# tensorflow/recommenders

Hardware: AMD Instinct MI355X
Metric: queries/sec brute-force top-100 (higher is better)
Workload: dtype f32; 1 GPU; BruteForce top-100, 1M-item x dim-64 corpus, batch 8192 (BASELINE.json configs[1]); corpus_rows_total=1000000, corpus_rows_per_gpu=1000000, dim=64, batch=8192, k=100, parallelism=single GPU

## Files before the change

recommenders_amd/csrc/topk_scan16.hip:

```cpp
#include <stdlib.h>

#include <string.h>

#include "common.h"

#ifndef TFRS_SCAN16_ABLATE
#define TFRS_SCAN16_ABLATE 0
#endif
#if TFRS_SCAN16_ABLATE
#ifndef TFRS_ALLOW_ABLATION
#error "TFRS_SCAN16_ABLATE != 0 is a measurement build with wrong results: add -DTFRS_ALLOW_ABLATION to confirm"
#endif
extern "C" int tfrs_ablation_build_scan16(void) { return TFRS_SCAN16_ABLATE; }
#endif
#ifndef TFRS_SCAN16_PEEL
#define TFRS_SCAN16_PEEL 2
#endif

#ifndef TFRS_SCAN16_CLOCKS
#define TFRS_SCAN16_CLOCKS 0
#endif

namespace tfrs {

typedef float f32x16 __attribute__((ext_vector_type(16)));
typedef float f32x4 __attribute__((ext_vector_type(4)));
typedef _Float16 f16x8 __attribute__((ext_vector_type(8)));
typedef _Float16 f16x2 __attribute__((ext_vector_type(2)));
typedef uint32_t u32x4 __attribute__((ext_vector_type(4)));

constexpr int kWaves16 = 8;
constexpr int kThreads16 = kWaves16 * 64;
constexpr int kQG = 2;
static_assert(kWaves16 * kQG * 32 == kScan16QueriesPerWg, "queries per workgroup");

enum Scan16Mode { kModeFilter = 0, kModeMaterialize = 1, kModeBinMax = 2 };

template <int DP>
struct Scan16Geom {
  static constexpr int kSteps = DP / 16;
  static constexpr int kRowB = DP * 2 + 16;
  static constexpr int kStageB = kTileN * kRowB;
  static constexpr int kChunks = kStageB / 16;
  static constexpr int kLoads = (kChunks + kThreads16 - 1) / kThreads16;
  static constexpr int kMetaOff = 2 * kStageB;
  static constexpr int kLdsBytes = 2 * kStageB + 32;
};


template <bool NT = false>
__device__ __forceinline__ void glds_copy16(const char *gsrc_lane, const char *lds_wave_base) {
  const uint32_t m0v = (uint32_t)(uintptr_t)(
      __attribute__((address_space(3))) const char *)lds_wave_base;
  uint32_t m0_saved;
  if constexpr (NT) {
    asm volatile("s_mov_b32 %0, m0\n\ts_mov_b32 m0, %2\n\ts_nop 0\n\t"
                 "global_load_lds_dwordx4 %1, off nt\n\ts_mov_b32 m0, %0"
                 : "=&s"(m0_saved)
                 : "v"(gsrc_lane), "s"(m0v)
                 : "memory");
  } else {
    asm volatile("s_mov_b32 %0, m0\n\ts_mov_b32 m0, %2\n\ts_nop 0\n\t"
                 "global_load_lds_dwordx4 %1, off\n\ts_mov_b32 m0, %0"
                 : "=&s"(m0_saved)
                 : "v"(gsrc_lane), "s"(m0v)
                 : "memory");
  }
}
__device__ __forceinline__ void wait_dma() {
  __builtin_amdgcn_s_waitcnt(0 | (7 << 4) | (15 << 8) | (0 << 14));
}

template <int CHUNKS, int LOADS, bool NT = false>
__device__ __forceinline__ void stage16_glds(const char *gsrc, char *lds_dst, const StageMeta *meta,
                                             char *lds_meta, int tid, int wave) {
#pragma unroll
  for (int i = 0; i < LOADS; ++i) {
    const int ch0 = i * kThreads16 + wave * 64;
    if (ch0 < CHUNKS)
      glds_copy16<NT>(gsrc + (size_t)(i * kThreads16 + tid) * 16, lds_dst + ch0 * 16);
  }
  if (tid == 0) glds_copy16(reinterpret_cast<const char *>(meta), lds_meta);
}

__device__ __forceinline__ f16x8 as_f16x8(u32x4 v) {
  union {
    u32x4 u;
    f16x8 b;
  } x;
  x.u = v;
  return x.b;
}
__device__ __forceinline__ uint32_t cvt_f16x2(float lo, float hi) {
  union {
    f16x2 h;
    uint32_t u;
  } v;
  v.h[0] = (_Float16)lo;
  v.h[1] = (_Float16)hi;
  return v.u;
}
__device__ __forceinline__ float mx3(float a, float b, float c) {
  return __builtin_fmaxf(__builtin_fmaxf(a, b), c);
}
__device__ __forceinline__ float max16(const f32x16 &c) {
  const float a = mx3(c[0], c[1], c[2]), b = mx3(c[3], c[4], c[5]), d = mx3(c[6], c[7], c[8]),
              e = mx3(c[9], c[10], c[11]), f = mx3(c[12], c[13], c[14]);
  return __builtin_fmaxf(mx3(a, b, d), mx3(e, f, c[15]));
}

__device__ __forceinline__ float max8(const f32x4 &c0, const f32x4 &c1) {
  return mx3(mx3(c0[0], c0[1], c0[2]), mx3(c0[3], c1[0], c1[1]), __builtin_fmaxf(c1[2], c1[3]));
}

template <int DP, int MF>
struct Scan16Mfma {
  static_assert(MF == 32 || (MF == 16 && DP >= 32), "the 16x16x32 shape needs 32 features per instruction");
  static constexpr int kQH = 32 / MF;
  static constexpr int kQW = MF;
  static constexpr int kKPer = 512 / MF;
  static constexpr int kKSteps = DP / kKPer;
  static constexpr int kFrags = DP / 16;
  static constexpr int kChain = kQH * kQH * kKSteps;
  static constexpr int kValuPerMfma = (MF == 16 && DP >= 64) ? 2 : 3;
  static constexpr int a_off(int sub, int m, int row_b) {
    return MF == 32 ? sub * 32 * row_b + m * 32
                    : (sub * 32 + 16 * (m / kKSteps)) * row_b + (m % kKSteps) * 64;
  }
};

template <int DP, int MODE, bool NT = false, int MF = 32>
__global__ void __launch_bounds__(kThreads16, DP <= 64 ? 4 : 2) scan16_kernel(const Scan16Args a) {
  using G = Scan16Geom<DP>;
  using M = Scan16Mfma<DP, MF>;
  static_assert(MF == 32 || MODE != kModeFilter, "the first-generation FILTER exists in the 32x32 shape only");
  constexpr int kNS = kQG * M::kQH;
  extern __shared__ __attribute__((aligned(16))) char smem[];

  const int tid = threadIdx.x;
  const int lane = tid & 63;
  const int wave = __builtin_amdgcn_readfirstlane(tid >> 6);
  if (MODE == kModeFilter && a.zero_word && blockIdx.x == 0 && tid == 0) *a.zero_word = 0u;
  if (MODE == kModeFilter && a.zero_aux && blockIdx.x == 0 && tid < 4) a.zero_aux[tid] = 0u;
  const int j = lane & (MF - 1);
  const int h = lane / MF;

  const int nwg = gridDim.x;
  const int bid = blockIdx.x;
  const int q8 = nwg >> 3, r8 = nwg & 7;
  const int xcd = bid & 7, pos = bid >> 3;
  const int logical = (xcd < r8 ? xcd * (q8 + 1) : r8 * (q8 + 1) + (xcd - r8) * q8) + pos;
  const int split = logical / a.n_qtiles;
  const int qt = logical - split * a.n_qtiles;

  const int i0 = split * a.stages_per_split;
  int i1 = i0 + a.stages_per_split;
  if (i1 > a.n_stages) i1 = a.n_stages;
  if (i0 >= i1) return;
  const int nst = i1 - i0;
  const int64_t stride = a.stage_stride;
  const int64_t first_stage = a.stage0 + (int64_t)i0 * stride;

  f16x8 bq[kNS][M::kKSteps];
  float lower[kNS], qk[kNS], qs[kNS], qinv[kNS];
  bool qvalid[kNS];
  int64_t qrow[kNS];
  uint2 *wp[kNS];
  uint32_t mycnt[kNS];
  const bool vec_ok = (a.d == DP) && ((reinterpret_cast<uintptr_t>(a.q) & 15) == 0);
  float4 qlo[kNS][M::kKSteps], qhi[kNS][M::kKSteps];
  int64_t qclampv[kNS];
#pragma unroll
  for (int g = 0; g < kNS; ++g) {
    qrow[g] = (int64_t)qt * kScan16QueriesPerWg + wave * (kQG * 32) + g * M::kQW + j;
    qvalid[g] = qrow[g] < a.nq;
    qclampv[g] = qvalid[g] ? qrow[g] : a.nq - 1;
    qs[g] = a.qscale[qclampv[g]];
  }
  if (vec_ok) {
#pragma unroll
    for (int g = 0; g < kNS; ++g) {
      const float *qp = a.q + qclampv[g] * a.d;
#pragma unroll
      for (int m = 0; m < M::kKSteps; ++m) {
        qlo[g][m] = *reinterpret_cast<const float4 *>(qp + M::kKPer * m + 8 * h);
        qhi[g][m] = *reinterpret_cast<const float4 *>(qp + M::kKPer * m + 8 * h + 4);
      }
    }
  }
#pragma unroll
  for (int g = 0; g < kNS; ++g) {
    const int64_t qclamp = qclampv[g];
    const float *qp = a.q + qclamp * a.d;
    if (!qvalid[g]) qs[g] = 1.0f;
    qinv[g] = 1.0f / qs[g];
#pragma unroll
    for (int m = 0; m < M::kKSteps; ++m) {
      float x[8];
      if (vec_ok) {
        float4 lo = qlo[g][m], hi = qhi[g][m];
        if (!qvalid[g]) lo = hi = make_float4(0.f, 0.f, 0.f, 0.f);
        x[0] = lo.x; x[1] = lo.y; x[2] = lo.z; x[3] = lo.w;
        x[4] = hi.x; x[5] = hi.y; x[6] = hi.z; x[7] = hi.w;
      } else {
#pragma unroll
        for (int i = 0; i < 8; ++i) {
          const int k = M::kKPer * m + 8 * h + i;
          x[i] = (qvalid[g] && k < a.d) ? qp[k] : 0.0f;
        }
      }
      u32x4 w;
#pragma unroll
      for (int i = 0; i < 4; ++i) w[i] = cvt_f16x2(x[2 * i] * qinv[g], x[2 * i + 1] * qinv[g]);
      bq[g][m] = as_f16x8(w);
    }
    lower[g] = __builtin_inff();
    qk[g] = 0.0f;
    if (MODE == kModeFilter) {
      const float lw = a.lower[qclamp], kq = a.qk[qclamp];
      lower[g] = qvalid[g] ? lw : __builtin_inff();
      qk[g] = qvalid[g] ? kq : 0.0f;
    }
    wp[g] = (MODE == kModeFilter)
                ? a.buf + (qrow[g] * (int64_t)a.cap_l) * a.nseg + (2 * split + h)
                : nullptr;
    mycnt[g] = 0;
  }
  const uint32_t row_limit = (uint32_t)a.row_limit;
  const bool wave_active =
      (int64_t)qt * kScan16QueriesPerWg + wave * (kQG * 32) < a.nq;

  static_assert(G::kChunks % 64 == 0, "stage size must be a whole number of wave copies");
  const char *gsrc = a.packed16 + first_stage * (int64_t)G::kStageB;
  const int64_t gstep = stride * (int64_t)G::kStageB;
  const StageMeta *mp = a.meta + first_stage;
  stage16_glds<G::kChunks, G::kLoads, NT>(gsrc, smem, mp, smem + G::kMetaOff, tid, wave);
  wait_dma();
  __syncthreads();

  float binmax[kNS];
#pragma unroll
  for (int g = 0; g < kNS; ++g) binmax[g] = -__builtin_inff();
  for (int st = 0; st < nst; ++st) {
    const char *tile = smem + (st & 1) * G::kStageB;
    const bool more = (st + 1 < nst);
    if (more) {
      stage16_glds<G::kChunks, G::kLoads, NT>(gsrc + (int64_t)(st + 1) * gstep,
                                          smem + ((st + 1) & 1) * G::kStageB,
                                          mp + (int64_t)(st + 1) * stride,
                                          smem + G::kMetaOff + ((st + 1) & 1) * 16, tid, wave);
    }
    const StageMeta sm = *reinterpret_cast<const StageMeta *>(smem + G::kMetaOff + (st & 1) * 16);
    float thr[kNS], unscale[kNS];
#pragma unroll
    for (int g = 0; g < kNS; ++g) {
      thr[g] = (__builtin_fmaf(-qk[g], sm.norm, lower[g]) - kF16Tiny) * qinv[g] * sm.inv_scale;
      unscale[g] = qs[g] * sm.scale;
    }
    if (MODE == kModeBinMax && (st % a.bin_stages) == 0) {
#pragma unroll
      for (int g = 0; g < kNS; ++g) binmax[g] = -__builtin_inff();
    }

    float stagemax[kNS];
#pragma unroll
    for (int g = 0; g < kNS; ++g) stagemax[g] = -__builtin_inff();
    const uint32_t stage_row = (uint32_t)((first_stage + (int64_t)st * stride) * kTileN);
    const char *ap = tile + j * G::kRowB + h * 16;

    if (!wave_active) goto stage_done;
    {
    u32x4 af[2][M::kFrags];
#pragma unroll
    for (int m = 0; m < M::kFrags; ++m) af[0][m] = *reinterpret_cast<const u32x4 *>(ap + M::a_off(0, m, G::kRowB));

    f32x16 acc[kQG];
    f32x4 acc4[kNS][2];
    auto chain = [&](int g, int sub) __attribute__((always_inline)) {
      if constexpr (MF == 16) {
#pragma unroll
        for (int qh = 0; qh < 2; ++qh)
#pragma unroll
          for (int ch = 0; ch < 2; ++ch) acc4[2 * g + qh][ch] = f32x4{0.0f, 0.0f, 0.0f, 0.0f};
#pragma unroll
        for (int m = 0; m < M::kKSteps; ++m)
#pragma unroll
          for (int qh = 0; qh < 2; ++qh)
#pragma unroll
            for (int ch = 0; ch < 2; ++ch)
              acc4[2 * g + qh][ch] = __builtin_amdgcn_mfma_f32_16x16x32_f16(
                  as_f16x8(af[sub & 1][ch * M::kKSteps + m]), bq[2 * g + qh][m], acc4[2 * g + qh][ch], 0, 0, 0);
        return;
      }
#pragma unroll
      for (int r = 0; r < 16; ++r) acc[g][r] = 0.0f;
#pragma unroll
      for (int m = 0; m < G::kSteps; ++m)
        acc[g] = __builtin_amdgcn_mfma_f32_32x32x16_f16(as_f16x8(af[sub & 1][m]), bq[g][m], acc[g], 0, 0, 0);
    };
    auto check = [&](int g, int sub) __attribute__((always_inline)) {
      if constexpr (MF == 16) {
#pragma unroll
        for (int qh = 0; qh < 2; ++qh) {
          const int s = 2 * g + qh;
          if (MODE == kModeMaterialize) {
            if (qvalid[s]) {
              float *drow = a.dense + qrow[s] * a.ld_dense + ((int64_t)(i0 + st) * kTileN + sub * 32 + 4 * h);
#pragma unroll
              for (int ch = 0; ch < 2; ++ch)
                *reinterpret_cast<float4 *>(drow + 16 * ch) =
                    make_float4(acc4[s][ch][0] * unscale[s], acc4[s][ch][1] * unscale[s],
                                acc4[s][ch][2] * unscale[s], acc4[s][ch][3] * unscale[s]);
            }
          } else {
            stagemax[s] = __builtin_fmaxf(stagemax[s], max8(acc4[s][0], acc4[s][1]));
            asm volatile("" : "+v"(stagemax[s]));
          }
        }
        return;
      }
      const f32x16 &c = acc[g];
      if (MODE == kModeMaterialize) {
        if (qvalid[g]) {
          float *drow = a.dense + qrow[g] * a.ld_dense +
                        ((int64_t)(i0 + st) * kTileN + sub * 32 + 4 * h);
#pragma unroll
          for (int g4 = 0; g4 < 4; ++g4)
            *reinterpret_cast<float4 *>(drow + 8 * g4) =
                make_float4(c[4 * g4 + 0] * unscale[g], c[4 * g4 + 1] * unscale[g],
                            c[4 * g4 + 2] * unscale[g], c[4 * g4 + 3] * unscale[g]);
        }
        return;
      }
      const float m0 = max16(c);
      if (MODE == kModeBinMax) {
        stagemax[g] = __builtin_fmaxf(stagemax[g], m0);
        asm volatile("" : "+v"(stagemax[g]));
        return;
      }
      if (__ballot(m0 > thr[g]) != 0ull) {
        const uint32_t rbase = stage_row + sub * 32 + 4u * h;
#pragma unroll
        for (int g4 = 0; g4 < 4; ++g4) {
          const float gm = __builtin_fmaxf(mx3(c[4 * g4], c[4 * g4 + 1], c[4 * g4 + 2]), c[4 * g4 + 3]);
          if (__ballot(gm > thr[g]) == 0ull) continue;
#pragma unroll
          for (int rr = 0; rr < 4; ++rr) {
            const float v = c[4 * g4 + rr];
            const uint32_t row = rbase + rr + 8 * g4;
            if (v > thr[g] && row < row_limit) {
              if (mycnt[g] < a.cap_l) *wp[g] = make_uint2(__float_as_uint(v * unscale[g]), row);
              wp[g] += a.nseg;
              ++mycnt[g];
            }
          }
        }
      }
    };
    auto interleave = [&]() __attribute__((always_inline)) {
#pragma unroll
      for (int i = 0; i < M::kChain; ++i) {
        __builtin_amdgcn_sched_group_barrier(0x008, 1, 0);
        __builtin_amdgcn_sched_group_barrier(0x002, M::kValuPerMfma, 0);
      }
    };

    chain(0, 0);
#pragma unroll
    for (int sub = 0; sub < kTileN / 32; ++sub) {
      if (sub + 1 < kTileN / 32) {
#pragma unroll
        for (int m = 0; m < M::kFrags; ++m)
          af[(sub + 1) & 1][m] =
              *reinterpret_cast<const u32x4 *>(ap + M::a_off(sub + 1, m, G::kRowB));
      }
      __builtin_amdgcn_sched_barrier(0);
      chain(1, sub);
      check(0, sub);
      if (MODE != kModeMaterialize) interleave();
      if (sub + 1 < kTileN / 32) {
        chain(0, sub + 1);
        check(1, sub);
        if (MODE != kModeMaterialize) interleave();
      } else {
        check(1, sub);
      }
    }
    }
  stage_done:
    if (MODE == kModeBinMax && wave_active) {
#pragma unroll
      for (int g = 0; g < kNS; ++g) binmax[g] = __builtin_fmaxf(binmax[g], stagemax[g] * unscale[g]);
      if ((st % a.bin_stages) == a.bin_stages - 1 || st == nst - 1) {
#pragma unroll
        for (int g = 0; g < kNS; ++g) {
          if constexpr (MF == 16) {
            const float v = __builtin_fmaxf(binmax[g], __shfl_xor(binmax[g], 16));
            if (qvalid[g] && (h & 1) == 0)
              a.binmax[qrow[g] * a.ld_binmax + 2 * ((i0 + st) / a.bin_stages) + (h >> 1)] = v;
          } else {
            if (qvalid[g])
              a.binmax[qrow[g] * a.ld_binmax + 2 * ((i0 + st) / a.bin_stages) + h] = binmax[g];
          }
        }
      }
    }
    wait_dma();
    __syncthreads();
  }

  if (MODE == kModeFilter) {
#pragma unroll
    for (int g = 0; g < kNS; ++g)
      if (qvalid[g]) a.cnt[qrow[g] * a.nseg + 2 * split + h] = mycnt[g];
  }
}


template <int DP, int NW, int QG, int SPB = 1, int MF = 32>
struct Scan16FGeom : Scan16Geom<DP> {
  using B = Scan16Geom<DP>;
  static constexpr int kTiles = NW * QG * 32 / kScan16QueriesPerWg;
  static constexpr int kWavesPerTile = NW / kTiles;
  static_assert(kTiles >= 1 && kTiles * kScan16QueriesPerWg == NW * QG * 32, "queries per workgroup");
  static constexpr int kThreads = NW * 64;
  static constexpr int kLoadsF = (B::kChunks + kThreads - 1) / kThreads;
  static constexpr int kQCap = 32;
  static constexpr int kEntB = MF == 16 ? 48 : 80;
  static constexpr int kWaveB = kQCap * kEntB + QG * 64 * 4 + QG * 64 * 16;
  static constexpr int kSlots = 2 * SPB;
  static constexpr int kMetaOffF = kSlots * B::kStageB;
  static constexpr int kQueueOff = (kMetaOffF + kSlots * 16 + 15) / 16 * 16;
  static constexpr int kLdsBytesF = kQueueOff + NW * kWaveB;
  static_assert(kLdsBytesF <= 160 * 1024, "LDS budget");
};

template <int CHUNKS, int LOADS, int THREADS, bool NT = false>
__device__ __forceinline__ void stage16f_glds(const char *gsrc, char *lds_dst, const StageMeta *meta,
                                              char *lds_meta, int tid, int wave) {
#pragma unroll
  for (int i = 0; i < LOADS; ++i) {
    const int ch0 = i * THREADS + wave * 64;
    if (ch0 < CHUNKS)
      glds_copy16<NT>(gsrc + (size_t)(i * THREADS + tid) * 16, lds_dst + ch0 * 16);
  }
  if (tid == 0) glds_copy16(reinterpret_cast<const char *>(meta), lds_meta);
}

__device__ __forceinline__ uint32_t lds_atomic_inc(uint32_t *p) {
  return __hip_atomic_fetch_add(p, 1u, __ATOMIC_RELAXED, __HIP_MEMORY_SCOPE_WAVEFRONT);
}


template <int DP, int NW, int QG, int SPB = 1, bool NT = false, int MF = 32>
__global__ void __launch_bounds__(NW * 64, NW * QG >= 32 ? 1 : (DP <= 64 ? 2 : 1) * NW / 4) scan16f_kernel(const Scan16Args a) {
  using G = Scan16FGeom<DP, NW, QG, SPB, MF>;
  using M = Scan16Mfma<DP, MF>;
  static_assert(MF == 32 || QG == 2, "the 16x16 shape is written for the two-group schedule");
  constexpr int kNS = QG * M::kQH;
  extern __shared__ __attribute__((aligned(16))) char smem[];

  const int tid = threadIdx.x;
  const int lane = tid & 63;
  const int wave = __builtin_amdgcn_readfirstlane(tid >> 6);
  if (a.zero_word && blockIdx.x == 0 && tid == 0) *a.zero_word = 0u;
  if (a.zero_aux && blockIdx.x == 0 && tid < 4) a.zero_aux[tid] = 0u;
  long long clk0 = 0, wall0 = 0;
  if (TFRS_SCAN16_CLOCKS) { clk0 = clock64(); wall0 = wall_clock64(); }
  const int j = lane & (MF - 1);
  const int h = lane / MF;
  const int tj = lane & 31;
  const int th = lane >> 5;

  const int nwg = gridDim.x;
  const int bid = blockIdx.x;
  const int q8 = nwg >> 3, r8 = nwg & 7;
  const int xcd = bid & 7, pos = bid >> 3;
  const int logical = (xcd < r8 ? xcd * (q8 + 1) : r8 * (q8 + 1) + (xcd - r8) * q8) + pos;
  const int n_qgroups = (a.n_qtiles + G::kTiles - 1) / G::kTiles;
  const int split = logical / n_qgroups;
  const int qt = (logical - split * n_qgroups) * G::kTiles + wave / G::kWavesPerTile;
  const int wave_in_tile = wave % G::kWavesPerTile;

  const int i0 = split * a.stages_per_split;
  int i1 = i0 + a.stages_per_split;
  if (i1 > a.n_stages) i1 = a.n_stages;
  if (i0 >= i1) return;
  const int nst = i1 - i0;
  const int64_t first_stage = a.stage0 + (int64_t)i0 * a.stage_stride;

  char *const qbase = smem + G::kQueueOff + wave * G::kWaveB;
  uint32_t *const wcnt = reinterpret_cast<uint32_t *>(qbase + G::kQCap * G::kEntB);
  #pragma unroll
  for (int g = 0; g < QG; ++g) wcnt[g * 64 + lane] = 0u;
  const int64_t q0 = (int64_t)qt * kScan16QueriesPerWg + wave_in_tile * (QG * 32);

  f16x8 bq[kNS][M::kKSteps];
  float4 *const qconst = reinterpret_cast<float4 *>(qbase + G::kQCap * G::kEntB + QG * 64 * 4);
  const bool vec_ok = (a.d == DP) && ((reinterpret_cast<uintptr_t>(a.q) & 15) == 0);
  float4 qlo[kNS][M::kKSteps], qhi[kNS][M::kKSteps];
  float qscv[QG], lowv[QG], qkv[QG];
  float qscb[kNS];
#pragma unroll
  for (int g = 0; g < QG; ++g) {
    const int64_t qrow = q0 + g * 32 + tj;
    const int64_t qclamp = qrow < a.nq ? qrow : a.nq - 1;
    qscv[g] = a.qscale[qclamp];
    lowv[g] = a.lower[qclamp];
    qkv[g] = a.qk[qclamp];
  }
  if constexpr (MF == 16) {
#pragma unroll
    for (int s = 0; s < kNS; ++s) {
      const int64_t qrow = q0 + s * M::kQW + j;
      qscb[s] = a.qscale[qrow < a.nq ? qrow : a.nq - 1];
    }
  }
  if (vec_ok) {
#pragma unroll
    for (int s = 0; s < kNS; ++s) {
      const int64_t qrow = q0 + s * M::kQW + j;
      const float *qp = a.q + (qrow < a.nq ? qrow : a.nq - 1) * a.d;
#pragma unroll
      for (int m = 0; m < M::kKSteps; ++m) {
        qlo[s][m] = *reinterpret_cast<const float4 *>(qp + M::kKPer * m + 8 * h);
        qhi[s][m] = *reinterpret_cast<const float4 *>(qp + M::kKPer * m + 8 * h + 4);
      }
    }
  }
#pragma unroll
  for (int s = 0; s < kNS; ++s) {
    const int64_t qrow = q0 + s * M::kQW + j;
    const bool qvalid = qrow < a.nq;
    const int64_t qclamp = qvalid ? qrow : a.nq - 1;
    const float *qp = a.q + qclamp * a.d;
    const float qsc = qvalid ? (MF == 16 ? qscb[s] : qscv[s / M::kQH]) : 1.0f;
    const float qinv = 1.0f / qsc;
#pragma unroll
    for (int m = 0; m < M::kKSteps; ++m) {
      float x[8];
      if (vec_ok) {
        float4 lo = qlo[s][m], hi = qhi[s][m];
        if (!qvalid) lo = hi = make_float4(0.f, 0.f, 0.f, 0.f);
        x[0] = lo.x; x[1] = lo.y; x[2] = lo.z; x[3] = lo.w;
        x[4] = hi.x; x[5] = hi.y; x[6] = hi.z; x[7] = hi.w;
      } else {
#pragma unroll
        for (int i = 0; i < 8; ++i) {
          const int k = M::kKPer * m + 8 * h + i;
          x[i] = (qvalid && k < a.d) ? qp[k] : 0.0f;
        }
      }
      u32x4 w;
#pragma unroll
      for (int i = 0; i < 4; ++i) w[i] = cvt_f16x2(x[2 * i] * qinv, x[2 * i + 1] * qinv);
      bq[s][m] = as_f16x8(w);
    }
  }
#pragma unroll
  for (int g = 0; g < QG; ++g) {
    const int64_t qrow = q0 + g * 32 + tj;
    const bool qvalid = qrow < a.nq;
    const float qsc = qvalid ? qscv[g] : 1.0f;
    const float lower_q = lowv[g], qk_q = qkv[g];
    const float qinv = 1.0f / qsc;
    const uint32_t seg_base = (uint32_t)((qrow * (int64_t)a.cap_l) * a.nseg + (2 * split + th));
    qconst[g * 64 + lane] = make_float4(qvalid ? (lower_q - kF16Tiny) * qinv : __builtin_inff(),
                                        qvalid ? qk_q * qinv : 0.0f, qsc,
                                        __uint_as_float(seg_base));
  }
  __builtin_amdgcn_fence(__ATOMIC_ACQ_REL, "wavefront");
  __builtin_amdgcn_wave_barrier();
  const uint32_t row_limit = (uint32_t)a.row_limit;
  const bool wave_active = q0 < a.nq;
  int qtail = 0;

  auto drain = [&]() __attribute__((always_inline)) {
    __builtin_amdgcn_fence(__ATOMIC_ACQ_REL, "wavefront");
    __builtin_amdgcn_wave_barrier();
    constexpr int kLanesPerEnt = MF == 16 ? 2 : 4;
    const uint32_t s4 = (uint32_t)(lane & (kLanesPerEnt - 1));
    for (int p0 = 0; p0 < qtail; p0 += 64 / kLanesPerEnt) {
      const int e = p0 + lane / kLanesPerEnt;
      if (e < qtail) {
        const char *ep = qbase + e * G::kEntB;
        const float4 v4 = *reinterpret_cast<const float4 *>(ep + 16 * s4);
        const uint4 hd = *reinterpret_cast<const uint4 *>(ep + G::kEntB - 16);
        const float thr_e = __uint_as_float(hd.x);
        const uint32_t row0 = hd.z + (MF == 16 ? 16u : 8u) * s4;
        uint32_t hits = (v4.x > thr_e ? 1u : 0u) | (v4.y > thr_e ? 2u : 0u) |
                        (v4.z > thr_e ? 4u : 0u) | (v4.w > thr_e ? 8u : 0u);
        if (row0 + 3u >= row_limit) {
#pragma unroll
          for (uint32_t i = 0; i < 4u; ++i)
            if (row0 + i >= row_limit) hits &= ~(1u << i);
        }
        if (hits) {
          const uint32_t src = hd.w;
          const float2 zc = *reinterpret_cast<const float2 *>(&qconst[src].z);
          const float un = zc.x * __uint_as_float(hd.y);
          do {
            const uint32_t i = (uint32_t)__builtin_ctz(hits);
            hits &= hits - 1u;
            const float v = i == 0u ? v4.x : i == 1u ? v4.y : i == 2u ? v4.z : v4.w;
            const uint32_t row = row0 + i;
            const uint32_t slot = lds_atomic_inc(&wcnt[src]);
            if (slot < a.cap_l) {
              a.buf[(uint64_t)(__float_as_uint(zc.y) + slot * (uint32_t)a.nseg)] =
                  make_uint2(__float_as_uint(v * un), row);
            } else if (a.ovf_cnt && slot - a.cap_l < kOvfPerSeg) {
              const int64_t qrow = q0 + (src >> 6) * 32 + (src & 31);
              const uint32_t o = atomicAdd(&a.ovf_cnt[qrow], 1u);
              if (o < a.ovf_cap) a.ovf_buf[qrow * (int64_t)a.ovf_cap + o] = make_uint2(__float_as_uint(v * un), row);
            }
          } while (hits);
        }
      }
    }
    __builtin_amdgcn_fence(__ATOMIC_ACQ_REL, "wavefront");
    __builtin_amdgcn_wave_barrier();
    qtail = 0;
  };

  static_assert(G::kChunks % 64 == 0, "stage size must be a whole number of wave copies");
  const char *gsrc = a.packed16 + first_stage * (int64_t)G::kStageB;
  const int64_t gstep = (int64_t)a.stage_stride * (int64_t)G::kStageB;
  const StageMeta *mp = a.meta + first_stage;
  auto copy_stage = [&](int st) __attribute__((always_inline)) {
    const int slot = ((st / SPB) & 1) * SPB + (st % SPB);
    stage16f_glds<G::kChunks, G::kLoadsF, G::kThreads, NT>(gsrc + (int64_t)st * gstep, smem + slot * G::kStageB,
                                                       mp + (int64_t)st * a.stage_stride,
                                                       smem + G::kMetaOffF + slot * 16, tid, wave);
  };
#pragma unroll
  for (int u = 0; u < SPB; ++u)
    if (u < nst) copy_stage(u);
  wait_dma();
  __syncthreads();

  const int n_periods = (nst + SPB - 1) / SPB;
  for (int per = 0; per < n_periods; ++per) {
    if (!((TFRS_SCAN16_ABLATE & 8) && per >= 1)) {
#pragma unroll
      for (int u = 0; u < SPB; ++u)
        if ((per + 1) * SPB + u < nst) copy_stage((per + 1) * SPB + u);
    }
#pragma unroll
    for (int u = 0; u < SPB; ++u) {
    const int st = per * SPB + u;
    if (SPB > 1 && st >= nst) break;
    const int slot = (per & 1) * SPB + u;
    const char *tile = smem + slot * G::kStageB;
    if (wave_active) {
    const StageMeta sm = *reinterpret_cast<const StageMeta *>(smem + G::kMetaOffF + slot * 16);
    const float s_norm = __uint_as_float(__builtin_amdgcn_readfirstlane(__float_as_uint(sm.norm)));
    const uint32_t s_scale_bits = __builtin_amdgcn_readfirstlane(__float_as_uint(sm.scale));
    const float s_inv = __uint_as_float(__builtin_amdgcn_readfirstlane(__float_as_uint(sm.inv_scale)));
    float thr[kNS];
#pragma unroll
    for (int s = 0; s < kNS; ++s) {
      const float4 qc = qconst[MF == 16 ? (s >> 1) * 64 + (s & 1) * 16 + j : s * 64 + lane];
      thr[s] = __builtin_fmaf(-qc.y, s_norm, qc.x) * s_inv;
    }
    const uint32_t stage_row = (uint32_t)((first_stage + (int64_t)st * a.stage_stride) * kTileN);
    const char *ap = tile + j * G::kRowB + h * 16;

    u32x4 af[2][M::kFrags];
#pragma unroll
    for (int m = 0; m < M::kFrags; ++m) af[0][m] = *reinterpret_cast<const u32x4 *>(ap + M::a_off(0, m, G::kRowB));

    f32x16 acc[QG];
    f32x4 acc4[kNS][2];
    if (TFRS_SCAN16_ABLATE & 32) __builtin_amdgcn_s_setprio(2);
    auto chain = [&](int g, int sub) __attribute__((always_inline)) {
      if constexpr (MF == 16) {
#pragma unroll
        for (int qh = 0; qh < 2; ++qh)
#pragma unroll
          for (int ch = 0; ch < 2; ++ch) acc4[2 * g + qh][ch] = f32x4{0.0f, 0.0f, 0.0f, 0.0f};
#pragma unroll
        for (int m = 0; m < M::kKSteps; ++m)
#pragma unroll
          for (int qh = 0; qh < 2; ++qh)
#pragma unroll
            for (int ch = 0; ch < 2; ++ch)
              acc4[2 * g + qh][ch] = __builtin_amdgcn_mfma_f32_16x16x32_f16(
                  as_f16x8(af[sub & 1][ch * M::kKSteps + m]), bq[2 * g + qh][m], acc4[2 * g + qh][ch], 0, 0, 0);
        return;
      }
#pragma unroll
      for (int r = 0; r < 16; ++r) acc[g][r] = 0.0f;
#pragma unroll
      for (int m = 0; m < G::kSteps; ++m)
        acc[g] = __builtin_amdgcn_mfma_f32_32x32x16_f16(as_f16x8(af[sub & 1][m]), bq[g][m], acc[g], 0, 0, 0);
    };
    auto check16 = [&](int g, int sub) __attribute__((always_inline)) {
      f32x4 (&c)[kNS][2] = acc4;
      if (TFRS_SCAN16_PEEL == 2)
        asm volatile("s_nop 7" : "+v"(c[2 * g][0]), "+v"(c[2 * g][1]), "+v"(c[2 * g + 1][0]), "+v"(c[2 * g + 1][1]));
      if (TFRS_SCAN16_ABLATE & 16) { asm volatile("" :: "v"(c[2 * g][0][0]), "v"(c[2 * g + 1][1][3])); return; }
      bool hot[2];
      uint64_t hm[2];
#pragma unroll
      for (int qh = 0; qh < 2; ++qh) {
        hot[qh] = max8(c[2 * g + qh][0], c[2 * g + qh][1]) > thr[2 * g + qh];
        hm[qh] = __ballot(hot[qh]);
      }
      if (TFRS_SCAN16_ABLATE & 2) { asm volatile("" :: "s"(hm[0]), "s"(hm[1])); return; }
      if (__builtin_expect((hm[0] | hm[1]) != 0ull, 0)) {
        const uint32_t rbase = stage_row + sub * 32 + 4u * h;
        auto put = [&](int qh, int slot) __attribute__((always_inline)) {
          char *e = qbase + slot * G::kEntB;
          const int s = 2 * g + qh;
          uint32_t src = (uint32_t)lane;
          asm volatile("" : "+v"(src));
          src = (src & 47u) + (uint32_t)(g * 64 + qh * 16);
#pragma unroll
          for (int ch = 0; ch < 2; ++ch)
            *reinterpret_cast<float4 *>(e + 16 * ch) = make_float4(c[s][ch][0], c[s][ch][1], c[s][ch][2], c[s][ch][3]);
          *reinterpret_cast<uint4 *>(e + 32) =
              make_uint4(__float_as_uint(thr[s]), s_scale_bits, rbase, src);
        };
        if (TFRS_SCAN16_PEEL) {
          const int n0 = __builtin_popcountll(hm[0]);
          const int nhot = n0 + __builtin_popcountll(hm[1]);
          if (__builtin_expect(qtail + nhot <= G::kQCap, 1)) {
#pragma unroll
            for (int qh = 0; qh < 2; ++qh)
              if (hot[qh])
                put(qh, qtail + (qh ? n0 : 0) + (int)__builtin_amdgcn_mbcnt_hi((uint32_t)(hm[qh] >> 32),
                                                     __builtin_amdgcn_mbcnt_lo((uint32_t)hm[qh], 0u)));
            qtail += nhot;
            return;
          }
        }
#pragma unroll
        for (int qh = 0; qh < 2; ++qh) {
          uint64_t rem = hm[qh];
          bool pending = hot[qh];
          while (__builtin_expect(rem != 0ull, 0)) {
            const int rank = (int)__builtin_amdgcn_mbcnt_hi((uint32_t)(rem >> 32),
                                 __builtin_amdgcn_mbcnt_lo((uint32_t)rem, 0u));
            const bool mine = pending && qtail + rank < G::kQCap;
            if (mine) put(qh, qtail + rank);
            pending = pending && !mine;
            qtail += __builtin_popcountll(__ballot(mine));
            rem = __ballot(pending);
            if (__builtin_expect(rem != 0ull, 0)) drain();
          }
        }
      }
    };
    auto check = [&](int g, int sub) __attribute__((always_inline)) {
      if constexpr (MF == 16) { check16(g, sub); return; }
      if (TFRS_SCAN16_PEEL == 2) asm volatile("s_nop 9" : "+v"(acc[g]));
      const f32x16 &c = acc[g];
      if (TFRS_SCAN16_ABLATE & 16) { asm volatile("" :: "v"(c[0]), "v"(c[15])); return; }
      const float m0 = max16(c);
      const bool hot = m0 > thr[g];
      const uint64_t hm = __ballot(hot);
      if (TFRS_SCAN16_ABLATE & 2) { asm volatile("" :: "s"(hm)); return; }
      if (__builtin_expect(hm != 0ull, 0)) {
        const uint32_t rbase = stage_row + sub * 32 + 4u * h;
        if (TFRS_SCAN16_PEEL) {
          const int nhot = __builtin_popcountll(hm);
          if (__builtin_expect(qtail + nhot <= G::kQCap, 1)) {
            if (hot) {
              const int rank = (int)__builtin_amdgcn_mbcnt_hi((uint32_t)(hm >> 32),
                                   __builtin_amdgcn_mbcnt_lo((uint32_t)hm, 0u));
              char *e = qbase + (qtail + rank) * G::kEntB;
#pragma unroll
              for (int g4 = 0; g4 < 4; ++g4)
                *reinterpret_cast<float4 *>(e + 16 * g4) =
                    make_float4(c[4 * g4], c[4 * g4 + 1], c[4 * g4 + 2], c[4 * g4 + 3]);
              *reinterpret_cast<uint4 *>(e + 64) =
                  make_uint4(__float_as_uint(thr[g]), s_scale_bits, rbase, (uint32_t)(g * 64 + lane));
            }
            qtail += nhot;
            return;
          }
        }
        uint64_t rem = hm;
        do {
          const int rank = (int)__builtin_amdgcn_mbcnt_hi((uint32_t)(rem >> 32),
                               __builtin_amdgcn_mbcnt_lo((uint32_t)rem, 0u));
          const bool mine = ((rem >> lane) & 1ull) != 0ull && qtail + rank < G::kQCap;
          if (mine) {
            char *e = qbase + (qtail + rank) * G::kEntB;
#pragma unroll
            for (int g4 = 0; g4 < 4; ++g4)
              *reinterpret_cast<float4 *>(e + 16 * g4) =
                  make_float4(c[4 * g4], c[4 * g4 + 1], c[4 * g4 + 2], c[4 * g4 + 3]);
            *reinterpret_cast<uint4 *>(e + 64) =
                make_uint4(__float_as_uint(thr[g]), s_scale_bits, rbase, (uint32_t)(g * 64 + lane));
          }
          const uint64_t taken = __ballot(mine);
          qtail += __builtin_popcountll(taken);
          rem &= ~taken;
          if (__builtin_expect(rem != 0ull, 0)) drain();
        } while (__builtin_expect(rem != 0ull, 0));
      }
    };
    auto interleave = [&]() __attribute__((always_inline)) {
#pragma unroll
      for (int i = 0; i < M::kChain; ++i) {
        __builtin_amdgcn_sched_group_barrier(0x008, 1, 0);
        __builtin_amdgcn_sched_group_barrier(0x002, M::kValuPerMfma, 0);
      }
    };

    if constexpr (QG == 2) {
    chain(0, 0);
#pragma unroll
    for (int sub = 0; sub < kTileN / 32; ++sub) {
      if (sub + 1 < kTileN / 32) {
#pragma unroll
        for (int m = 0; m < M::kFrags; ++m)
          if (TFRS_SCAN16_ABLATE & 4) af[(sub + 1) & 1][m] = af[sub & 1][m];
          else
          af[(sub + 1) & 1][m] =
              *reinterpret_cast<const u32x4 *>(ap + M::a_off(sub + 1, m, G::kRowB));
      }
      __builtin_amdgcn_sched_barrier(0);
      chain(1, sub);
      check(0, sub);
      interleave();
      if (sub + 1 < kTileN / 32) {
        chain(0, sub + 1);
        check(1, sub);
        interleave();
      } else {
        check(1, sub);
      }
    }
    } else {
#pragma unroll
    for (int sub = 0; sub < kTileN / 32; ++sub) {
      if (sub + 1 < kTileN / 32) {
#pragma unroll
        for (int m = 0; m < G::kSteps; ++m)
          af[(sub + 1) & 1][m] =
              *reinterpret_cast<const u32x4 *>(ap + (sub + 1) * 32 * G::kRowB + m * 32);
      }
      __builtin_amdgcn_sched_barrier(0);
#pragma unroll
      for (int g = 0; g < QG; ++g) {
        chain(g, sub);
        if (g > 0) {
          check(g - 1, sub);
          interleave();
        } else if (sub > 0) {
          check(QG - 1, sub - 1);
          interleave();
        }
      }
    }
    check(QG - 1, kTileN / 32 - 1);
    }
    }
    }
    if (TFRS_SCAN16_ABLATE & 32) __builtin_amdgcn_s_setprio(0);
    wait_dma();
    if (qtail > 0 && (qtail >= a.drain_min || per == n_periods - 1 || ((per + 1) % a.drain_every) == 0)) drain();
    if (!(TFRS_SCAN16_ABLATE & 1)) __builtin_amdgcn_s_barrier();
  }

  __builtin_amdgcn_fence(__ATOMIC_ACQ_REL, "wavefront");
  __builtin_amdgcn_wave_barrier();
  int ln = lane;
  asm volatile("" : "+v"(ln));
#pragma unroll
  for (int g = 0; g < QG; ++g) {
    const int64_t qrow = q0 + g * 32 + (ln & 31);
    if (qrow < a.nq) a.cnt[qrow * a.nseg + 2 * split + (ln >> 5)] = wcnt[g * 64 + ln];
  }
#if TFRS_SCAN16_CLOCKS
  if (blockIdx.x == 0 && tid == 0)
    printf("scan16f_clocks mfma %d dim %d cycles %lld ticks100MHz %lld\n", MF, DP, clock64() - clk0, wall_clock64() - wall0);
#endif
}


static bool scan16_nt_copies(const Scan16Args &a) {
  const char *e = option("TFRS_SCAN16_NT");
  return a.n_qtiles == 1 && !(e && e[0] == '0');
}

template <int DP>
constexpr bool kScan16Has16x16 = DP >= 32 && TFRS_SCAN16_PEEL != 1;
constexpr int scan16_default_mfma(int dp) { return dp >= 64 ? 16 : 32; }

static int scan16_mfma(int dp, int *mf) {
  const char *e = option("TFRS_SCAN16_MFMA");
  *mf = scan16_default_mfma(dp);
  if (e) {
    if (strcmp(e, "32x32") == 0) *mf = 32;
    else if (strcmp(e, "16x16") == 0) *mf = 16;
    else {
      set_error("TFRS_SCAN16_MFMA=%s: expected 32x32 or 16x16", e);
      return TFRS_EINVAL;
    }
  }
  return TFRS_OK;
}

template <int DP, int NW, int QG, int SPB = 1, bool NT = false, int MF = 32>
static int launch_scan16f(const Scan16Args &a, hipStream_t stream) {
  using G = Scan16FGeom<DP, NW, QG, SPB, MF>;
  TFRS_HIP(ensure_dynamic_lds(reinterpret_cast<const void *>(&scan16f_kernel<DP, NW, QG, SPB, NT, MF>), G::kLdsBytesF));
  const dim3 grid((unsigned)((a.n_qtiles + G::kTiles - 1) / G::kTiles * a.n_splits));
  hipLaunchKernelGGL((scan16f_kernel<DP, NW, QG, SPB, NT, MF>), grid, dim3(NW * 64), G::kLdsBytesF, stream, a);
  TFRS_LAUNCH_CHECK();
  return TFRS_OK;
}

template <int DP, int NW, int QG, int SPB = 1, bool NT = false>
static int launch_scan16f_mf(const Scan16Args &a, hipStream_t stream, int mf) {
  if constexpr (kScan16Has16x16<DP>) {
    if (mf == 16) return launch_scan16f<DP, NW, QG, SPB, NT, 16>(a, stream);
  }
  return launch_scan16f<DP, NW, QG, SPB, NT, 32>(a, stream);
}

template <int DP>
static int launch_scan16f_shape(const Scan16Args &a, hipStream_t stream) {
  const char *e = option("TFRS_SCAN16_SHAPE");
  const bool pair = a.n_qtiles >= 2;
  auto is = [&](const char *v) { return e && strcmp(e, v) == 0; };
  if (e && !(is("16x2s2") || is("16x2") || is("8x2") || is("4x4") || is("8x4"))) {
    set_error("TFRS_SCAN16_SHAPE=%s: expected one of 16x2s2, 16x2, 8x2, 4x4, 8x4", e);
    return TFRS_EINVAL;
  }
  int mf;
  if (const int rc = scan16_mfma(DP, &mf)) return rc;
  if (is("8x2")) return launch_scan16f_mf<DP, 8, 2>(a, stream, mf);
  if constexpr (DP <= 64) {
    if (is("4x4")) return launch_scan16f<DP, 4, 4>(a, stream);
    if (is("8x4") && pair) return launch_scan16f<DP, 8, 4>(a, stream);
    if (is("16x2") && pair) return launch_scan16f<DP, 16, 2>(a, stream);
    if (pair) return launch_scan16f_mf<DP, 16, 2, 2>(a, stream, mf);
  }
  if (!e && scan16_nt_copies(a)) return launch_scan16f_mf<DP, 8, 2, 1, true>(a, stream, mf);
  return launch_scan16f_mf<DP, 8, 2>(a, stream, mf);
}

template <int DP, int MODE, bool NT = false, int MF = 32>
static int launch_scan16_variant(const Scan16Args &a, hipStream_t stream) {
  using G = Scan16Geom<DP>;
  if constexpr (MODE == kModeBinMax && !NT) {
    if (scan16_nt_copies(a)) return launch_scan16_variant<DP, MODE, true, MF>(a, stream);
  }
  TFRS_HIP(ensure_dynamic_lds(reinterpret_cast<const void *>(&scan16_kernel<DP, MODE, NT, MF>), G::kLdsBytes));
  const dim3 grid((unsigned)(a.n_qtiles * a.n_splits));
  hipLaunchKernelGGL((scan16_kernel<DP, MODE, NT, MF>), grid, dim3(kThreads16), G::kLdsBytes, stream, a);
  TFRS_LAUNCH_CHECK();
  return TFRS_OK;
}

template <int DP>
static int launch_scan16_dp(const Scan16Args &a, hipStream_t stream) {
  if (a.dense || a.binmax) {
    int mf;
    if (const int rc = scan16_mfma(DP, &mf)) return rc;
    if constexpr (kScan16Has16x16<DP>) {
      if (mf == 16)
        return a.dense ? launch_scan16_variant<DP, kModeMaterialize, false, 16>(a, stream)
                       : launch_scan16_variant<DP, kModeBinMax, false, 16>(a, stream);
    }
    return a.dense ? launch_scan16_variant<DP, kModeMaterialize>(a, stream)
                   : launch_scan16_variant<DP, kModeBinMax>(a, stream);
  }
  return launch_scan16_variant<DP, kModeFilter>(a, stream);
}

static int scan16_generation() {
  const char *e = option("TFRS_SCAN16_V");
  return (e && e[0] == '1') ? 1 : 2;
}

int launch_scan16(const Scan16Args &a_in, hipStream_t stream) {
  Scan16Args a = a_in;
  if (a.nq <= 0 || a.n_stages <= 0) return TFRS_OK;
  if (a.drain_min < 1) a.drain_min = 1;
  if (a.drain_every < 1) a.drain_every = 1;
  TFRS_CHECK_ARG(a.stage_stride >= 1 && a.stages_per_split >= 1 &&
                     (int64_t)a.n_splits * a.stages_per_split >= a.n_stages,
                 "scan16: bad stage split");
  TFRS_CHECK_ARG(a.dense || a.binmax || a.nseg == 2 * a.n_splits, "scan16: nseg must be 2 * n_splits");
  TFRS_CHECK_ARG(!a.binmax || (a.bin_stages >= 1 && a.stages_per_split % a.bin_stages == 0),
                 "scan16: stages_per_split must be a multiple of bin_stages");
  const bool fits32 = (uint64_t)a.nq * a.cap_l * (uint64_t)a.nseg < (1ull << 32);
  if (!a.dense && !a.binmax && fits32 && scan16_generation() == 2) {
    switch (padded_dim16(a.d)) {
      case 16: return launch_scan16f_shape<16>(a, stream);
      case 32: return launch_scan16f_shape<32>(a, stream);
      case 64: return launch_scan16f_shape<64>(a, stream);
      case 128: return launch_scan16f_shape<128>(a, stream);
    }
  }
  switch (padded_dim16(a.d)) {
    case 16: return launch_scan16_dp<16>(a, stream);
    case 32: return launch_scan16_dp<32>(a, stream);
    case 64: return launch_scan16_dp<64>(a, stream);
    case 128: return launch_scan16_dp<128>(a, stream);
  }
  set_error("scan16: unsupported dim %d", a.d);
  return TFRS_ENOTIMPL;
}

}
```

Before: 7.693 million queries/s.

## Stagger next-stage LDS DMA copies inside the MFMA loop and load stage metadata via scalar loads

The copy of the next corpus stage into LDS now uses a scalar base address with per-lane offsets, and it is issued inside the MFMA sub-tile loop. Each group of four waves issues its copy at a different sub-tile, so the DMA traffic is spread across the compute instead of bunched at the start of each stage. Stage metadata is no longer copied into LDS. It is prefetched one stage ahead through constant-address-space scalar loads, which also removes the readfirstlane calls and frees the LDS meta slots. The change adds optional timestamp instrumentation, and it risks scheduling interference and extra SGPR pressure in the hot loop.

```diff
diff --git a/recommenders_amd/csrc/topk_scan16.hip b/recommenders_amd/csrc/topk_scan16.hip
--- a/recommenders_amd/csrc/topk_scan16.hip
+++ b/recommenders_amd/csrc/topk_scan16.hip
@@ -19,6 +19,16 @@
 
 #ifndef TFRS_SCAN16_CLOCKS
 #define TFRS_SCAN16_CLOCKS 0
+#endif
+
+#ifndef TFRS_SCAN16_COPY
+#define TFRS_SCAN16_COPY 1
+#endif
+#ifndef TFRS_SCAN16_COPY_FILTER
+#define TFRS_SCAN16_COPY_FILTER TFRS_SCAN16_COPY
+#endif
+#ifndef TFRS_SCAN16_COPY_THRESHOLD
+#define TFRS_SCAN16_COPY_THRESHOLD TFRS_SCAN16_COPY
 #endif
 
 namespace tfrs {
@@ -67,6 +77,114 @@
                  : "memory");
   }
 }
+template <bool NT = false>
+__device__ __forceinline__ void glds_copy16s(const char *gsrc_wave, uint32_t lane_off, const char *lds_wave_base) {
+  const uint32_t m0v = (uint32_t)(uintptr_t)(
+      __attribute__((address_space(3))) const char *)lds_wave_base;
+  uint32_t m0_saved;
+  if constexpr (NT) {
+    asm volatile("s_mov_b32 %0, m0\n\ts_mov_b32 m0, %3\n\ts_nop 0\n\t"
+                 "global_load_lds_dwordx4 %1, %2 nt\n\ts_mov_b32 m0, %0"
+                 : "=&s"(m0_saved)
+                 : "v"(lane_off), "s"(gsrc_wave), "s"(m0v)
+                 : "memory");
+  } else {
+    asm volatile("s_mov_b32 %0, m0\n\ts_mov_b32 m0, %3\n\ts_nop 0\n\t"
+                 "global_load_lds_dwordx4 %1, %2\n\ts_mov_b32 m0, %0"
+                 : "=&s"(m0_saved)
+                 : "v"(lane_off), "s"(gsrc_wave), "s"(m0v)
+                 : "memory");
+  }
+}
+template <int CHUNKS, int LOADS, int THREADS, bool NT = false>
+__device__ __forceinline__ void stage16_glds_s(const char *gsrc, char *lds_dst, uint32_t lane_off, int wave) {
+#pragma unroll
+  for (int i = 0; i < LOADS; ++i) {
+    const int ch0 = i * THREADS + wave * 64;
+    if ((i + 1) * THREADS <= CHUNKS || ch0 < CHUNKS)
+      glds_copy16s<NT>(gsrc + (size_t)ch0 * 16, lane_off, lds_dst + ch0 * 16);
+  }
+}
+__device__ __forceinline__ int opaque_s(int v) {
+  asm volatile("" : "+s"(v));
+  return v;
+}
+__device__ __forceinline__ const char *opaque_s(const char *v) {
+  asm volatile("" : "+s"(v));
+  return v;
+}
+__device__ __forceinline__ StageMeta stage_meta_k(const StageMeta *p) {
+  const f32x4 v = *(const __attribute__((address_space(4))) f32x4 *)(uintptr_t)p;
+  StageMeta m;
+  m.norm = v[0];
+  m.scale = v[1];
+  m.inv_scale = v[2];
+  m.pad_ = 0.0f;
+  return m;
+}
+#if TFRS_SCAN16_CLOCKS
+__device__ unsigned long long g_scan16_stamps[2][16][8];
+__device__ __forceinline__ unsigned long long stamp16() {
+  unsigned long long t;
+  __builtin_amdgcn_sched_barrier(0);
+  asm volatile("s_memtime %0\n\ts_waitcnt lgkmcnt(0)" : "=s"(t) :: "memory");
+  __builtin_amdgcn_sched_barrier(0);
+  return t;
+}
+#endif
+struct Scan16Stamps {
+#if TFRS_SCAN16_CLOCKS
+  unsigned long long t_copy = 0, n_blocks = 0, n_pieces = 0, t_head = 0, n_periods = 0, n_stamps = 0;
+  unsigned long long t_loop = 0, w_loop = 0, s_bar = 0, s_tmp = 0;
+#endif
+  __device__ __forceinline__ void loop_begin() {
+#if TFRS_SCAN16_CLOCKS
+    t_copy = n_blocks = n_pieces = 0;
+    w_loop = __builtin_amdgcn_s_memrealtime();
+    t_loop = stamp16();
+#endif
+  }
+  __device__ __forceinline__ void loop_end(int kernel, int wave, int lane) {
+#if TFRS_SCAN16_CLOCKS
+    t_loop = stamp16() - t_loop;
+    w_loop = __builtin_amdgcn_s_memrealtime() - w_loop;
+    __builtin_amdgcn_s_waitcnt(0xC07F);
+    if (blockIdx.x == 0 && lane == 0 && wave < 16) {
+      unsigned long long *o = g_scan16_stamps[kernel][wave];
+      o[0] = t_copy; o[1] = n_blocks; o[2] = n_pieces; o[3] = t_head;
+      o[4] = n_periods; o[5] = t_loop; o[6] = w_loop; o[7] = n_stamps;
+    }
+#endif
+  }
+  __device__ __forceinline__ void period_begin() {
+#if TFRS_SCAN16_CLOCKS
+    s_bar = stamp16(); ++n_periods; ++n_stamps;
+#endif
+  }
+  __device__ __forceinline__ void first_mfma() {
+#if TFRS_SCAN16_CLOCKS
+    t_head += stamp16() - s_bar; ++n_stamps;
+#endif
+  }
+  __device__ __forceinline__ void copy_begin() {
+#if TFRS_SCAN16_CLOCKS
+    s_tmp = stamp16(); ++n_stamps;
+#endif
+  }
+  __device__ __forceinline__ void copy_end(int pieces) {
+#if TFRS_SCAN16_CLOCKS
+    t_copy += stamp16() - s_tmp; ++n_blocks; n_pieces += (unsigned)pieces; ++n_stamps;
+#endif
+  }
+};
+template <int CHUNKS, int LOADS, int THREADS>
+__device__ __forceinline__ int stage16_pieces(int wave) {
+  int n = 0;
+#pragma unroll
+  for (int i = 0; i < LOADS; ++i) n += (i * THREADS + wave * 64 < CHUNKS) ? 1 : 0;
+  return n;
+}
+
 __device__ __forceinline__ void wait_dma() {
   __builtin_amdgcn_s_waitcnt(0 | (7 << 4) | (15 << 8) | (0 << 14));
 }
@@ -234,9 +352,24 @@
   const char *gsrc = a.packed16 + first_stage * (int64_t)G::kStageB;
   const int64_t gstep = stride * (int64_t)G::kStageB;
   const StageMeta *mp = a.meta + first_stage;
-  stage16_glds<G::kChunks, G::kLoads, NT>(gsrc, smem, mp, smem + G::kMetaOff, tid, wave);
+  constexpr bool kCopyInLoop = TFRS_SCAN16_COPY_THRESHOLD != 0;
+  const uint32_t lane_off = (uint32_t)lane * 16u;
+  auto copy_stage = [&](int s, int w, const char *src) __attribute__((always_inline)) {
+    if constexpr (kCopyInLoop)
+      stage16_glds_s<G::kChunks, G::kLoads, kThreads16, NT>(src, smem + (s & 1) * G::kStageB, lane_off, w);
+    else
+      stage16_glds<G::kChunks, G::kLoads, NT>(gsrc + (int64_t)s * gstep, smem + (s & 1) * G::kStageB,
+                                              mp + (int64_t)s * stride, smem + G::kMetaOff + (s & 1) * 16, tid, w);
+  };
+  Scan16Stamps stamps;
+  const int my_pieces = stage16_pieces<G::kChunks, G::kLoads, kThreads16>(wave) + ((!kCopyInLoop && wave == 0) ? 1 : 0);
+  copy_stage(0, wave, gsrc);
+  const char *gnext = gsrc + gstep;
+  StageMeta sm_next = {};
+  if constexpr (kCopyInLoop) sm_next = stage_meta_k(mp);
   wait_dma();
   __syncthreads();
+  stamps.loop_begin();
 
   float binmax[kNS];
 #pragma unroll
@@ -244,13 +377,19 @@
   for (int st = 0; st < nst; ++st) {
     const char *tile = smem + (st & 1) * G::kStageB;
     const bool more = (st + 1 < nst);
-    if (more) {
-      stage16_glds<G::kChunks, G::kLoads, NT>(gsrc + (int64_t)(st + 1) * gstep,
-                                          smem + ((st + 1) & 1) * G::kStageB,
-                                          mp + (int64_t)(st + 1) * stride,
-                                          smem + G::kMetaOff + ((st + 1) & 1) * 16, tid, wave);
-    }
-    const StageMeta sm = *reinterpret_cast<const StageMeta *>(smem + G::kMetaOff + (st & 1) * 16);
+    stamps.period_begin();
+    if (more && (!kCopyInLoop || !wave_active)) {
+      stamps.copy_begin();
+      copy_stage(st + 1, wave, gnext);
+      stamps.copy_end(my_pieces);
+    }
+    StageMeta sm;
+    if constexpr (kCopyInLoop) {
+      sm = sm_next;
+      sm_next = stage_meta_k(mp + (int64_t)(more ? st + 1 : st) * stride);
+    } else {
+      sm = *reinterpret_cast<const StageMeta *>(smem + G::kMetaOff + (st & 1) * 16);
+    }
     float thr[kNS], unscale[kNS];
 #pragma unroll
     for (int g = 0; g < kNS; ++g) {
@@ -365,6 +504,7 @@
       }
     };
 
+    stamps.first_mfma();
     chain(0, 0);
 #pragma unroll
     for (int sub = 0; sub < kTileN / 32; ++sub) {
@@ -375,6 +515,16 @@
               *reinterpret_cast<const u32x4 *>(ap + M::a_off(sub + 1, m, G::kRowB));
       }
       __builtin_amdgcn_sched_barrier(0);
+      if constexpr (kCopyInLoop) {
+        if (sub < kWaves16 / 4 && more) {
+          const int w = opaque_s(wave);
+          if ((w >> 2) == sub) {
+            stamps.copy_begin();
+            copy_stage(opaque_s(st) + 1, w, opaque_s(gnext));
+            stamps.copy_end(my_pieces);
+          }
+        }
+      }
       chain(1, sub);
       check(0, sub);
       if (MODE != kModeMaterialize) interleave();
@@ -407,7 +557,9 @@
     }
     wait_dma();
     __syncthreads();
-  }
+    gnext += gstep;
+  }
+  stamps.loop_end(1, wave, lane);
 
   if (MODE == kModeFilter) {
 #pragma unroll
@@ -430,7 +582,8 @@
   static constexpr int kWaveB = kQCap * kEntB + QG * 64 * 4 + QG * 64 * 16;
   static constexpr int kSlots = 2 * SPB;
   static constexpr int kMetaOffF = kSlots * B::kStageB;
-  static constexpr int kQueueOff = (kMetaOffF + kSlots * 16 + 15) / 16 * 16;
+  static constexpr int kMetaSlots = TFRS_SCAN16_COPY_FILTER ? 0 : kSlots;
+  static constexpr int kQueueOff = (kMetaOffF + kMetaSlots * 16 + 15) / 16 * 16;
   static constexpr int kLdsBytesF = kQueueOff + NW * kWaveB;
   static_assert(kLdsBytesF <= 160 * 1024, "LDS budget");
 };
@@ -626,24 +779,54 @@
   const char *gsrc = a.packed16 + first_stage * (int64_t)G::kStageB;
   const int64_t gstep = (int64_t)a.stage_stride * (int64_t)G::kStageB;
   const StageMeta *mp = a.meta + first_stage;
-  auto copy_stage = [&](int st) __attribute__((always_inline)) {
-    const int slot = ((st / SPB) & 1) * SPB + (st % SPB);
-    stage16f_glds<G::kChunks, G::kLoadsF, G::kThreads, NT>(gsrc + (int64_t)st * gstep, smem + slot * G::kStageB,
-                                                       mp + (int64_t)st * a.stage_stride,
-                                                       smem + G::kMetaOffF + slot * 16, tid, wave);
+  constexpr bool kCopyInLoop = TFRS_SCAN16_COPY_FILTER != 0;
+  static_assert(NW / 4 <= kTileN / 32, "one sub-tile of the first stage per wave of a SIMD");
+  const uint32_t lane_off = (uint32_t)lane * 16u;
+  auto copy_stage = [&](int p, int u, int w, const char *src) __attribute__((always_inline)) {
+    const int st = p * SPB + u;
+    const int slot = (p & 1) * SPB + u;
+    if constexpr (kCopyInLoop)
+      stage16_glds_s<G::kChunks, G::kLoadsF, G::kThreads, NT>(src + u * gstep, smem + slot * G::kStageB, lane_off, w);
+    else
+      stage16f_glds<G::kChunks, G::kLoadsF, G::kThreads, NT>(gsrc + (int64_t)st * gstep, smem + slot * G::kStageB,
+                                                         mp + (int64_t)st * a.stage_stride,
+                                                         smem + G::kMetaOffF + slot * 16, tid, w);
   };
-#pragma unroll
-  for (int u = 0; u < SPB; ++u)
-    if (u < nst) copy_stage(u);
+  Scan16Stamps stamps;
+  const int my_pieces = stage16_pieces<G::kChunks, G::kLoadsF, G::kThreads>(wave) + ((!kCopyInLoop && wave == 0) ? 1 : 0);
+  auto copy_period = [&](int p, int w, const char *src) __attribute__((always_inline)) {
+    if ((TFRS_SCAN16_ABLATE & 8) && p >= 2) return;
+    stamps.copy_begin();
+    int issued = 0;
+#pragma unroll
+    for (int u = 0; u < SPB; ++u)
+      if (p * SPB + u < nst) { copy_stage(p, u, w, src); issued += my_pieces; }
+    stamps.copy_end(issued);
+  };
+  auto meta_of = [&](int st) __attribute__((always_inline)) {
+    return stage_meta_k(mp + (int64_t)(st < nst ? st : nst - 1) * a.stage_stride);
+  };
+  copy_period(0, wave, gsrc);
+  const char *gnext = gsrc + SPB * gstep;
+  StageMeta smk[SPB], smk_next[SPB];
+  if constexpr (kCopyInLoop) {
+#pragma unroll
+    for (int u = 0; u < SPB; ++u) smk_next[u] = meta_of(u);
+  }
   wait_dma();
   __syncthreads();
+  stamps.loop_begin();
 
   const int n_periods = (nst + SPB - 1) / SPB;
   for (int per = 0; per < n_periods; ++per) {
-    if (!((TFRS_SCAN16_ABLATE & 8) && per >= 1)) {
-#pragma unroll
-      for (int u = 0; u < SPB; ++u)
-        if ((per + 1) * SPB + u < nst) copy_stage((per + 1) * SPB + u);
+    stamps.period_begin();
+    if (!kCopyInLoop || !wave_active) copy_period(per + 1, wave, gnext);
+    if constexpr (kCopyInLoop) {
+#pragma unroll
+      for (int u = 0; u < SPB; ++u) {
+        smk[u] = smk_next[u];
+        smk_next[u] = meta_of((per + 1) * SPB + u);
+      }
     }
 #pragma unroll
     for (int u = 0; u < SPB; ++u) {
@@ -652,10 +835,18 @@
     const int slot = (per & 1) * SPB + u;
     const char *tile = smem + slot * G::kStageB;
     if (wave_active) {
-    const StageMeta sm = *reinterpret_cast<const StageMeta *>(smem + G::kMetaOffF + slot * 16);
-    const float s_norm = __uint_as_float(__builtin_amdgcn_readfirstlane(__float_as_uint(sm.norm)));
-    const uint32_t s_scale_bits = __builtin_amdgcn_readfirstlane(__float_as_uint(sm.scale));
-    const float s_inv = __uint_as_float(__builtin_amdgcn_readfirstlane(__float_as_uint(sm.inv_scale)));
+    float s_norm, s_inv;
+    uint32_t s_scale_bits;
+    if constexpr (kCopyInLoop) {
+      s_norm = smk[u].norm;
+      s_scale_bits = __float_as_uint(smk[u].scale);
+      s_inv = smk[u].inv_scale;
+    } else {
+      const StageMeta sm = *reinterpret_cast<const StageMeta *>(smem + G::kMetaOffF + slot * 16);
+      s_norm = __uint_as_float(__builtin_amdgcn_readfirstlane(__float_as_uint(sm.norm)));
+      s_scale_bits = __builtin_amdgcn_readfirstlane(__float_as_uint(sm.scale));
+      s_inv = __uint_as_float(__builtin_amdgcn_readfirstlane(__float_as_uint(sm.inv_scale)));
+    }
     float thr[kNS];
 #pragma unroll
     for (int s = 0; s < kNS; ++s) {
@@ -810,6 +1001,7 @@
     };
 
     if constexpr (QG == 2) {
+    if (u == 0) stamps.first_mfma();
     chain(0, 0);
 #pragma unroll
     for (int sub = 0; sub < kTileN / 32; ++sub) {
@@ -822,6 +1014,12 @@
               *reinterpret_cast<const u32x4 *>(ap + M::a_off(sub + 1, m, G::kRowB));
       }
       __builtin_amdgcn_sched_barrier(0);
+      if constexpr (kCopyInLoop) {
+        if (u == 0 && sub < NW / 4) {
+          const int w = opaque_s(wave);
+          if ((w >> 2) == sub) copy_period(opaque_s(per) + 1, w, opaque_s(gnext));
+        }
+      }
       chain(1, sub);
       check(0, sub);
       interleave();
@@ -843,6 +1041,12 @@
               *reinterpret_cast<const u32x4 *>(ap + (sub + 1) * 32 * G::kRowB + m * 32);
       }
       __builtin_amdgcn_sched_barrier(0);
+      if constexpr (kCopyInLoop) {
+        if (u == 0 && sub < NW / 4) {
+          const int w = opaque_s(wave);
+          if ((w >> 2) == sub) copy_period(opaque_s(per) + 1, w, opaque_s(gnext));
+        }
+      }
 #pragma unroll
       for (int g = 0; g < QG; ++g) {
         chain(g, sub);
@@ -863,7 +1067,9 @@
     wait_dma();
     if (qtail > 0 && (qtail >= a.drain_min || per == n_periods - 1 || ((per + 1) % a.drain_every) == 0)) drain();
     if (!(TFRS_SCAN16_ABLATE & 1)) __builtin_amdgcn_s_barrier();
-  }
+    gnext += SPB * gstep;
+  }
+  stamps.loop_end(0, wave, lane);
 
   __builtin_amdgcn_fence(__ATOMIC_ACQ_REL, "wavefront");
   __builtin_amdgcn_wave_barrier();
@@ -1009,3 +1215,9 @@
 }
 
 }
+
+#if TFRS_SCAN16_CLOCKS
+extern "C" int tfrs_scan16_stamps_read(unsigned long long *out) {
+  return hipMemcpyFromSymbol(out, HIP_SYMBOL(tfrs::g_scan16_stamps), sizeof(tfrs::g_scan16_stamps)) == hipSuccess ? 0 : 1;
+}
+#endif
```

Result: no change. 7.692 million queries/s (median of 3 runs) (-0.0%).
